# LitLeo/3m-asr-inference

Hardware: AMD Instinct MI355X
Metric: encoder frames/sec, 18Lx32e Conformer-MoE, 206-frame utterance (higher is better)
Workload: dtype f32; 1 GPU; 18-layer 32-expert fp32 (v_mfma_f32_16x16x4_f32), batch=1x206 frames per GPU, all experts local (BASELINE.json configs[1]); layers=18, experts=32, frames=206, batch_per_gpu=1, parallelism=replicas x1, streams_per_gpu=4, hip_graph=True, kernels_per_forward=263, fold_pos_proj=True, routing=balanced, route_mode=staged, packed_rows=False, fork_embed=auto

## Files before the change

### 3m-asr-inference_amd/csrc/gemm.hip

```cpp
#include "common.h"
#include "gemm_epilogue.h"
#include "kernels.h"

#ifdef M3_GEMM_DIAG
#define M3_GDIAG(...) __VA_ARGS__
#else
#define M3_GDIAG(...)
#endif

namespace m3 {

M3_GDIAG(__device__ unsigned long long g_gemm_dbg[2048 * 8];)

enum { LN_NONE = GEMM_LN_NONE, LN_EPI = GEMM_LN_EPI, LN_PRO = GEMM_LN_PRO };

template <int MT, bool GLU, int NW, bool CONV, int LN, int NBUF, bool ACCI = false, bool WF = false>
__device__ __forceinline__ void gemm_f32_body(const GemmParams& p, const int bid) {
  static_assert(!WF || (!CONV && !ACCI), "fragment-ordered W: plain A only");
  constexpr int NT = GLU ? 2 : 1;
  constexpr int G = gemm_group_steps(MT, NT, NW);
  constexpr int I0 = ACCI ? G / 2 : 0;
  static_assert(!ACCI || (MT == 1 && !GLU && !CONV && NBUF == 1 && G % 2 == 0), "acc_init: the one-group 16-row concat form only");
  constexpr int RW = (16 * MT) / NW;
  static_assert(RW >= 1, "more waves than rows");
  __shared__ float red[NW][MT * NT][256];
  __shared__ float stats[16 * MT][2];
  __shared__ float rsum[LN == LN_EPI ? NW : 1][16 * MT][2];
  __shared__ __attribute__((aligned(16))) float ln_g[LN == LN_PRO ? 1024 : 4], ln_b[LN == LN_PRO ? 1024 : 4];

  M3_GDIAG(unsigned long long dg[8]; dg[0] = __builtin_amdgcn_s_memtime();)
  asm volatile("" ::"s"(p.A), "s"(p.lda), "s"(p.W), "s"(p.bias), "s"(p.Y), "s"(p.ldy), "s"(p.M), "s"(p.N), "s"(p.K), "s"(p.mode),
               "s"(p.n_tiles), "s"(p.m_tiles), "s"(p.xcd_swizzle), "s"(p.m_dev), "s"(p.resid), "s"(p.ldr), "s"(p.act), "s"(p.alpha),
               "s"(p.mask_in), "s"(p.mask_out), "s"(p.row_len), "s"(p.rows_per_batch), "s"(p.sig_col0));
  if (ACCI) asm volatile("" ::"s"(p.acc_init));
  if (LN == LN_EPI) asm volatile("" ::"s"(p.ln_wsum), "s"(p.ln_wbeta), "s"(p.ln_eps));
  if (LN == LN_PRO) asm volatile("" ::"s"(p.ln_gamma), "s"(p.ln_beta), "s"(p.ln_eps), "s"(p.ln_out), "s"(p.ld_ln_out), "s"(p.ln_on_a2));
  if (!CONV) asm volatile("" ::"s"(p.A2), "s"(p.lda2), "s"(p.K1));
  if (CONV) asm volatile("" ::"s"(p.conv_T1), "s"(p.conv_F1), "s"(p.conv_T2), "s"(p.conv_F2), "s"(p.conv_C));
  const int lane = threadIdx.x & 63, wave = threadIdx.x >> 6;
  const int col = lane & 15, kq = lane >> 4;
  const int Nout = GLU ? (p.N >> 1) : p.N;

  int n_tile, m_tile;
  {
    const int id = bid;
    if (p.xcd_swizzle) {
      const int j = id >> 3;
      m_tile = j % p.m_tiles;
      n_tile = (j / p.m_tiles) * 8 + (id & 7);
    } else {
      n_tile = id % p.n_tiles;
      m_tile = id / p.n_tiles;
    }
  }
  const int n0 = n_tile * 16;
  const int m0 = m_tile * (16 * MT);
  if (p.m_dev != nullptr && m0 > *p.m_dev) return;
  const int ln_k0 = p.ln_on_a2 ? p.K1 : 0;
  const int Kl = p.K - ln_k0;

  const float* arow[MT];
  const float* arow2[MT];
#pragma unroll
  for (int mt = 0; mt < MT; ++mt) {
    const int m = min(m0 + 16 * mt + col, p.M - 1);
    arow2[mt] = nullptr;
    if (CONV) {
      const int f2 = m % p.conv_F2;
      const int t2 = (m / p.conv_F2) % p.conv_T2;
      const int b = m / (p.conv_F2 * p.conv_T2);
      arow[mt] = p.A + ((size_t)(b * p.conv_T1 + 2 * t2) * p.conv_F1 + 2 * f2) * p.conv_C + 4 * kq;
    } else {
      arow[mt] = p.A + (size_t)m * p.lda + 4 * kq;
      if (p.mode == GEMM_A_CONCAT2) arow2[mt] = p.A2 + (size_t)m * p.lda2 + 4 * kq;
    }
  }
  const float* wrow[NT];
#pragma unroll
  for (int t = 0; t < NT; ++t)
    wrow[t] = WF ? p.W + (size_t)(n_tile + t * (Nout >> 4)) * ((size_t)p.K << 4) + 4 * lane
                 : p.W + (size_t)min(n0 + t * Nout + col, p.N - 1) * p.K + 4 * kq;

  f32x4 acc[MT][NT];
#pragma unroll
  for (int mt = 0; mt < MT; ++mt)
#pragma unroll
    for (int t = 0; t < NT; ++t) acc[mt][t] = f32x4{0.f, 0.f, 0.f, 0.f};
  constexpr bool DUAL = MT * NT <= 2;
  f32x4 acc2[MT][NT];
#pragma unroll
  for (int mt = 0; mt < MT; ++mt)
#pragma unroll
    for (int t = 0; t < NT; ++t) acc2[mt][t] = f32x4{0.f, 0.f, 0.f, 0.f};
  float s1[MT], s2[MT];
#pragma unroll
  for (int mt = 0; mt < MT; ++mt) s1[mt] = s2[mt] = 0.f;

  const int nsteps = p.K >> 4;
  auto a_offset = [&](int k) -> int {
    if (CONV) {
      const int seg = k / p.conv_C, c = k - seg * p.conv_C;
      const int kh = seg / 3, kw = seg - kh * 3;
      return (kh * p.conv_F1 + kw) * p.conv_C + c;
    }
    return k;
  };

  f32x4 wbuf[NBUF][G][NT], abuf[NBUF][G][MT];
  auto load_group = [&](int g, int buf) {
#pragma unroll
    for (int i = I0; i < G; ++i) {
      const int s = min(wave + NW * (G * g + i), nsteps - 1);
      const int k = s << 4;
#pragma unroll
      for (int t = 0; t < NT; ++t) wbuf[buf][i][t] = ldg4_w(wrow[t] + (WF ? (s << 8) : k));
      const bool second = ACCI || (!CONV && p.mode == GEMM_A_CONCAT2 && k >= p.K1);
      const int off = second ? (k - p.K1) : a_offset(k);
#pragma unroll
      for (int mt = 0; mt < MT; ++mt) abuf[buf][i][mt] = ldg4((second ? arow2[mt] : arow[mt]) + off);
    }
  };

  const int ngroups = (nsteps + NW * G - 1) / (NW * G);
  M3_GDIAG(dg[1] = __builtin_amdgcn_s_memtime();)
  f32x4 ln_v[16];
  auto load_stat_rows = [&](int c) {
    const int l16 = lane & 15;
    const int rloc = wave * RW + 4 * c + (lane >> 4);
    const int m = min(m0 + min(rloc, 16 * MT - 1), p.M - 1);
    const float* row = (p.ln_on_a2 ? p.A2 : p.A) + (size_t)m * (p.ln_on_a2 ? p.lda2 : p.lda);
#pragma unroll
    for (int j = 0; j < 8; ++j) ln_v[j] = ldg4(row + min(4 * (l16 + 16 * j), Kl - 4));
    if (Kl > 512) {
#pragma unroll
      for (int j = 8; j < 16; ++j) ln_v[j] = ldg4(row + min(4 * (l16 + 16 * j), Kl - 4));
    } else {
#pragma unroll
      for (int j = 8; j < 16; ++j) ln_v[j] = f32x4{0.f, 0.f, 0.f, 0.f};
    }
  };
  if (LN == LN_PRO && ACCI) load_stat_rows(0);
  load_group(0, 0);
  if (ACCI) {
    const float* pre = p.acc_init + ((size_t)((m_tile * p.n_tiles + n_tile) * NW + wave) * 2) * 256 + 4 * lane;
    acc[0][0] = ldg4(pre);
    acc2[0][0] = ldg4(pre + 256);
  }
  M3_GDIAG(dg[2] = __builtin_amdgcn_s_memtime();)
  const int ep_mt = wave;
  const bool is_ep = wave < MT;
  const int ep_n = n0 + col;
  float bias0 = 0.f, bias1 = 0.f, wsum0 = 0.f, wsum1 = 0.f, wbeta0 = 0.f, wbeta1 = 0.f, res[4] = {0.f, 0.f, 0.f, 0.f};
  if (is_ep && ep_n < Nout) {
    if (p.bias) {
      bias0 = p.bias[ep_n];
      if (GLU) bias1 = p.bias[ep_n + Nout];
    }
    if (LN == LN_EPI) {
      wsum0 = p.ln_wsum[ep_n];
      if (GLU) wsum1 = p.ln_wsum[ep_n + Nout];
      if (p.mask_in) {
        wbeta0 = p.ln_wbeta[ep_n];
        if (GLU) wbeta1 = p.ln_wbeta[ep_n + Nout];
      }
    }
    if (p.resid) {
#pragma unroll
      for (int r = 0; r < 4; ++r) {
        const int m = min(m0 + 16 * ep_mt + 4 * kq + r, p.M - 1);
        res[r] = p.resid[(size_t)m * p.ldr + ep_n];
      }
    }
  }
  bool pad4[4] = {false, false, false, false};
  if (is_ep && (p.mask_in || p.mask_out)) {
#pragma unroll
    for (int r = 0; r < 4; ++r) {
      const int m = min(m0 + 16 * ep_mt + 4 * kq + r, p.M - 1);
      pad4[r] = gemm_row_padded(p, m);
    }
  }


  float a_mean[MT], a_rstd[MT];
  float* ln_out_row[MT];
#pragma unroll
  for (int mt = 0; mt < MT; ++mt) {
    a_mean[mt] = 0.f;
    a_rstd[mt] = 1.f;
    ln_out_row[mt] = nullptr;
  }
  if (LN == LN_PRO) {
    for (int k = threadIdx.x * 4; k < Kl; k += 256 * NW) {
      *reinterpret_cast<f32x4*>(&ln_g[k]) = ldg4(p.ln_gamma + k);
      *reinterpret_cast<f32x4*>(&ln_b[k]) = ldg4(p.ln_beta + k);
    }
    const int q = lane >> 4, l16 = lane & 15;
    const int nj = (Kl + 63) >> 6;
    for (int c = 0; c < (RW + 3) / 4; ++c) {
      const int rloc = wave * RW + 4 * c + q;
      const bool row_on = (4 * c + q) < RW;
      f32x4 v[16];
      if (!(ACCI && c == 0)) load_stat_rows(c);
#pragma unroll
      for (int j = 0; j < 16; ++j) {
        const int k = 4 * (l16 + 16 * j);
        const f32x4 t = ln_v[j];
        const bool in = j < nj && k < Kl;
        v[j] = f32x4{in ? t[0] : 0.f, in ? t[1] : 0.f, in ? t[2] : 0.f, in ? t[3] : 0.f};
      }
      float sum = 0.f;
#pragma unroll
      for (int j = 0; j < 16; ++j) sum += (v[j][0] + v[j][1]) + (v[j][2] + v[j][3]);
      const float mean = group16_sum(sum) / (float)Kl;
      float sq = 0.f;
#pragma unroll
      for (int j = 0; j < 16; ++j) {
        const int k = 4 * (l16 + 16 * j);
        const float on = (j < nj && k < Kl) ? 1.f : 0.f;
#pragma unroll
        for (int e = 0; e < 4; ++e) {
          const float d = (v[j][e] - mean) * on;
          sq += d * d;
        }
      }
      const float var = group16_sum(sq) / (float)Kl;
      if (row_on && l16 == 0) {
        stats[rloc][0] = mean;
        stats[rloc][1] = rsqrtf(var + p.ln_eps);
      }
    }
    __syncthreads();
#pragma unroll
    for (int mt = 0; mt < MT; ++mt) {
      a_mean[mt] = stats[16 * mt + col][0];
      a_rstd[mt] = stats[16 * mt + col][1];
      const int m = m0 + 16 * mt + col;
      if (p.ln_out != nullptr && n_tile == 0 && m < p.M) ln_out_row[mt] = p.ln_out + (size_t)m * p.ld_ln_out + 4 * kq;
    }
  }

  auto compute_group = [&](int g, int buf) {
#pragma unroll
    for (int i = I0; i < G; ++i) {
      const int s = wave + NW * (G * g + i);
      if (s < nsteps) {
        const int k = s << 4;
        const bool in_ln = k >= ln_k0;
        f32x4 g4, b4;
        if (LN == LN_PRO && in_ln) {
          g4 = *reinterpret_cast<const f32x4*>(&ln_g[(k - ln_k0) + 4 * kq]);
          b4 = *reinterpret_cast<const f32x4*>(&ln_b[(k - ln_k0) + 4 * kq]);
        }
#pragma unroll
        for (int mt = 0; mt < MT; ++mt) {
          f32x4 a = abuf[buf][i][mt];
          if (LN == LN_PRO && in_ln) {
#pragma unroll
            for (int j = 0; j < 4; ++j) a[j] = (a[j] - a_mean[mt]) * a_rstd[mt] * g4[j] + b4[j];
            if (ln_out_row[mt] != nullptr) stg4(ln_out_row[mt] + (k - ln_k0), a);
          }
          if (LN == LN_EPI && in_ln) {
            s1[mt] += (a[0] + a[1]) + (a[2] + a[3]);
            s2[mt] += (a[0] * a[0] + a[1] * a[1]) + (a[2] * a[2] + a[3] * a[3]);
          }
#pragma unroll
          for (int t = 0; t < NT; ++t) {
            if (DUAL) {
#pragma unroll
              for (int j = 0; j < 4; j += 2) {
                acc[mt][t] = mfma16(a[j], wbuf[buf][i][t][j], acc[mt][t]);
                acc2[mt][t] = mfma16(a[j + 1], wbuf[buf][i][t][j + 1], acc2[mt][t]);
              }
            } else {
#pragma unroll
              for (int j = 0; j < 4; ++j) acc[mt][t] = mfma16(a[j], wbuf[buf][i][t][j], acc[mt][t]);
            }
          }
        }
      }
    }
  };

  M3_GDIAG(asm volatile("s_waitcnt vmcnt(0)" ::: "memory"); dg[3] = __builtin_amdgcn_s_memtime();)
  if (NBUF == 1) {
    compute_group(0, 0);
  } else {
    for (int g = 0; g < ngroups; g += 2) {
      if (g + 1 < ngroups) load_group(g + 1, NBUF - 1);
      compute_group(g, 0);
      if (g + 1 < ngroups) {
        if (g + 2 < ngroups) load_group(g + 2, 0);
        compute_group(g + 1, NBUF - 1);
      }
    }
  }

  if (DUAL) {
#pragma unroll
    for (int mt = 0; mt < MT; ++mt)
#pragma unroll
      for (int t = 0; t < NT; ++t) acc[mt][t] += acc2[mt][t];
  }
  M3_GDIAG(asm volatile("s_nop 15\n\ts_nop 15" ::: "memory"); dg[4] = __builtin_amdgcn_s_memtime();)
#pragma unroll
  for (int mt = 0; mt < MT; ++mt)
#pragma unroll
    for (int t = 0; t < NT; ++t)
#pragma unroll
      for (int r = 0; r < 4; ++r) red[wave][mt * NT + t][r * 64 + lane] = acc[mt][t][r];
  if (LN == LN_EPI) {
#pragma unroll
    for (int mt = 0; mt < MT; ++mt) {
      float a1 = s1[mt], a2 = s2[mt];
      a1 += __shfl_xor(a1, 16, 64);
      a2 += __shfl_xor(a2, 16, 64);
      a1 += __shfl_xor(a1, 32, 64);
      a2 += __shfl_xor(a2, 32, 64);
      if (kq == 0) {
        rsum[wave][16 * mt + col][0] = a1;
        rsum[wave][16 * mt + col][1] = a2;
      }
    }
  }
  __syncthreads();
  M3_GDIAG(dg[5] = __builtin_amdgcn_s_memtime();)

  if (is_ep) {
    const int mt = ep_mt;
    f32x4 v[NT];
#pragma unroll
    for (int t = 0; t < NT; ++t)
#pragma unroll
      for (int r = 0; r < 4; ++r) {
        float sum = 0.f;
#pragma unroll
        for (int w = 0; w < NW; w += 4)
          sum += (red[w][mt * NT + t][r * 64 + lane] + red[w + 1][mt * NT + t][r * 64 + lane]) +
                 (red[w + 2][mt * NT + t][r * 64 + lane] + red[w + 3][mt * NT + t][r * 64 + lane]);
        v[t][r] = sum;
      }
    if (ep_n < Nout) {
#pragma unroll
      for (int r = 0; r < 4; ++r) {
        const int row = 16 * mt + 4 * kq + r;
        const int m = m0 + row;
        if (m >= p.M) continue;
        float y0 = v[0][r], y1 = v[NT - 1][r];
        const bool pad = pad4[r];
        if (LN != LN_EPI && p.mask_in && pad) y0 = y1 = 0.f;
        float mean = 0.f, rstd = 1.f;
        if (LN == LN_EPI) {
          float t1 = 0.f, t2 = 0.f;
#pragma unroll
          for (int w = 0; w < NW; ++w) {
            t1 += rsum[w][row][0];
            t2 += rsum[w][row][1];
          }
          ln_mean_rstd(t1, t2, Kl, p.ln_eps, mean, rstd);
        }
        float y = gemm_epilogue<GLU, LN == LN_EPI>(y0, y1, bias0, bias1, wsum0, wsum1, wbeta0, wbeta1, mean, rstd, pad, res[r], p);
        if (!GLU && p.sig_col0 >= 0 && n0 >= p.sig_col0) y = sigmoidf(y);
        p.Y[(size_t)m * p.ldy + ep_n] = y;
      }
    }
  }
  M3_GDIAG(dg[6] = __builtin_amdgcn_s_memtime();
           asm volatile("s_waitcnt vmcnt(0)" ::: "memory");
           dg[7] = __builtin_amdgcn_s_memtime();
           if (lane == 0 && wave == 0 && bid < 2048) {
             unsigned long long* o = g_gemm_dbg + (size_t)bid * 8;
             for (int i = 0; i < 8; ++i) o[i] = dg[i];
             const unsigned hw = __builtin_amdgcn_s_getreg((31 << 11) | 4), xcc = __builtin_amdgcn_s_getreg((31 << 11) | 20);
             o[7] = (dg[7] & 0xffffffffffull) | ((unsigned long long)(hw & 0xffff) << 40) | ((unsigned long long)(xcc & 0xf) << 56);
           })
}

template <int MT, bool GLU, int NW, bool CONV, int LN, int NBUF, bool ACCI = false, bool WF = false>
__global__ __launch_bounds__(64 * NW) void gemm_f32_kernel(const GemmParams p) {
  gemm_f32_body<MT, GLU, NW, CONV, LN, NBUF, ACCI, WF>(p, (int)blockIdx.x);
}

struct RouterPrefixArgs {
  const float* A; int lda; int M, N, K;
  int n_tiles, m_tiles, xcd_swizzle;
  const int32_t* m_dev;
  float* prefix; long layer_floats; int layer0;
  const float* w[kRouterPrefixMaxLayers];
};
template <int NW>
__global__ __launch_bounds__(64 * NW) void router_embed_prefix_kernel(const RouterPrefixArgs a) {
  constexpr int H = gemm_group_steps(1, 1, NW) / 2;
  asm volatile("" ::"s"(a.A), "s"(a.lda), "s"(a.M), "s"(a.N), "s"(a.K), "s"(a.n_tiles), "s"(a.m_tiles), "s"(a.xcd_swizzle), "s"(a.m_dev),
               "s"(a.prefix), "s"(a.layer_floats), "s"(a.layer0));
  const int lane = threadIdx.x & 63, wave = threadIdx.x >> 6;
  const int col = lane & 15, kq = lane >> 4;
  const int layer = a.layer0 + (int)blockIdx.y;
  int n_tile, m_tile;
  {
    const int id = (int)blockIdx.x;
    if (a.xcd_swizzle) {
      const int j = id >> 3;
      m_tile = j % a.m_tiles;
      n_tile = (j / a.m_tiles) * 8 + (id & 7);
    } else {
      n_tile = id % a.n_tiles;
      m_tile = id / a.n_tiles;
    }
  }
  const int n0 = n_tile * 16, m0 = m_tile * 16;
  if (a.m_dev != nullptr && m0 > *a.m_dev) return;
  const float* arow = a.A + (size_t)min(m0 + col, a.M - 1) * a.lda + 4 * kq;
  const float* wrow = a.w[layer] + (size_t)min(n0 + col, a.N - 1) * a.K + 4 * kq;
  f32x4 wb[H], ab[H];
#pragma unroll
  for (int i = 0; i < H; ++i) {
    const int k = (wave + NW * i) << 4;
    wb[i] = ldg4_w(wrow + k);
    ab[i] = ldg4(arow + k);
  }
  f32x4 acc = f32x4{0.f, 0.f, 0.f, 0.f}, acc2 = f32x4{0.f, 0.f, 0.f, 0.f};
#pragma unroll
  for (int i = 0; i < H; ++i)
#pragma unroll
    for (int j = 0; j < 4; j += 2) {
      acc = mfma16(ab[i][j], wb[i][j], acc);
      acc2 = mfma16(ab[i][j + 1], wb[i][j + 1], acc2);
    }
  float* o = a.prefix + (size_t)layer * a.layer_floats + ((size_t)((m_tile * a.n_tiles + n_tile) * NW + wave) * 2) * 256 + 4 * lane;
  stg4(o, acc);
  stg4(o + 256, acc2);
}

size_t router_prefix_floats(const GemmPlan& plan) { return (size_t)plan.m_tiles * plan.n_tiles * plan.nw * 2 * 256; }

int launch_router_embed_prefix(const GemmPlan& plan, const GemmParams& p, const float* const* w, int layer0, int n_layers, float* prefix,
                               hipStream_t stream) {
  M3_REQUIRE(plan.launches == 1 && plan.kernel == GemmKernel::SkinnyF32 && p.acc_init != nullptr && (plan.nw == 4 || plan.nw == 8),
             "router prefix: the consumer's plan does not take an accumulator prefix");
  M3_REQUIRE(layer0 >= 0 && n_layers > 0 && layer0 + n_layers <= kRouterPrefixMaxLayers && prefix != nullptr, "router prefix: bad layer range");
  RouterPrefixArgs a;
  a.A = p.A; a.lda = p.lda; a.M = p.M; a.N = p.N; a.K = p.K;
  a.n_tiles = plan.n_tiles; a.m_tiles = plan.m_tiles; a.xcd_swizzle = plan.xcd_swizzle;
  a.m_dev = p.m_dev; a.prefix = prefix; a.layer_floats = (long)router_prefix_floats(plan); a.layer0 = layer0;
  for (int l = 0; l < kRouterPrefixMaxLayers; ++l) a.w[l] = (l >= layer0 && l < layer0 + n_layers) ? w[l] : nullptr;
  const dim3 grid(plan.n_tiles * plan.m_tiles, n_layers);
  if (plan.nw == 8) hipLaunchKernelGGL((router_embed_prefix_kernel<8>), grid, dim3(512), 0, stream, a);
  else hipLaunchKernelGGL((router_embed_prefix_kernel<4>), grid, dim3(256), 0, stream, a);
  M3_LAUNCH_CHECK();
  return 0;
}
template <int MT, bool GLU, int NW, int LN, bool WF = false>
__global__ __launch_bounds__(64 * NW) void gemm_f32_dual_kernel(const GemmParams p0, const GemmParams p1, const int n0) {
  if ((int)blockIdx.x < n0) {
    if ((int)blockIdx.x < p0.n_tiles * p0.m_tiles) gemm_f32_body<MT, GLU, NW, false, LN, 1, false, WF>(p0, (int)blockIdx.x);
  } else {
    gemm_f32_body<MT, GLU, NW, false, LN, 1, false, WF>(p1, (int)blockIdx.x - n0);
  }
}

int launch_gemm_f32_dual(const GemmLaunch& a, const GemmLaunch& b, hipStream_t stream) {
  M3_REQUIRE(gemm_dual_fusable(a, b), "gemm dual: the two problems do not share an instantiation");
  GemmParams q[2] = {a.p, b.p};
  const GemmPlan& pa = a.plan;
  const GemmPlan* const plans[2] = {&a.plan, &b.plan};
  for (int i = 0; i < 2; ++i) {
    q[i].n_tiles = plans[i]->n_tiles; q[i].m_tiles = plans[i]->m_tiles; q[i].xcd_swizzle = plans[i]->xcd_swizzle;
  }
  const int n0 = (int)align_up((size_t)q[0].n_tiles * q[0].m_tiles, 8);
  dim3 grid(n0 + q[1].n_tiles * q[1].m_tiles);
#define M3_DUAL(GLU_, NW_, LN_)                                                                                             \
  do {                                                                                                                      \
    if (q[0].w_frag) hipLaunchKernelGGL((gemm_f32_dual_kernel<1, GLU_, NW_, LN_, true>), grid, dim3(64 * NW_), 0, stream, q[0], q[1], n0); \
    else hipLaunchKernelGGL((gemm_f32_dual_kernel<1, GLU_, NW_, LN_>), grid, dim3(64 * NW_), 0, stream, q[0], q[1], n0);    \
  } while (0)
  if (pa.glu) {
    if (pa.nw == 8) { if (pa.ln == LN_EPI) M3_DUAL(true, 8, LN_EPI); else M3_DUAL(true, 8, LN_NONE); }
    else { if (pa.ln == LN_EPI) M3_DUAL(true, 4, LN_EPI); else M3_DUAL(true, 4, LN_NONE); }
  } else {
    if (pa.nw == 8) { if (pa.ln == LN_EPI) M3_DUAL(false, 8, LN_EPI); else M3_DUAL(false, 8, LN_NONE); }
    else { if (pa.ln == LN_EPI) M3_DUAL(false, 4, LN_EPI); else M3_DUAL(false, 4, LN_NONE); }
  }
#undef M3_DUAL
  M3_LAUNCH_CHECK();
  return 0;
}

int launch_gemm_f32_skinny(const GemmPlan& plan, const GemmParams& pin, hipStream_t stream) {
  GemmParams p = pin;
  p.n_tiles = plan.n_tiles; p.m_tiles = plan.m_tiles; p.xcd_swizzle = plan.xcd_swizzle;
  dim3 grid(p.n_tiles * p.m_tiles);
  const int mt = plan.mt, nw = plan.nw, ln = plan.ln;
  if (p.acc_init != nullptr) {
    if (nw == 8) hipLaunchKernelGGL((gemm_f32_kernel<1, false, 8, false, LN_PRO, 1, true>), grid, dim3(512), 0, stream, p);
    else hipLaunchKernelGGL((gemm_f32_kernel<1, false, 4, false, LN_PRO, 1, true>), grid, dim3(256), 0, stream, p);
    M3_LAUNCH_CHECK();
    return 0;
  }

#define M3_GEMM_LAUNCH(MT_, GLU_, NW_, CONV_, LN_)                                                              \
  do {                                                                                                          \
    constexpr bool kWf = !(CONV_);         \
    if (p.w_frag && plan.nbuf == 1)                                                                              \
      hipLaunchKernelGGL((gemm_f32_kernel<MT_, GLU_, NW_, CONV_, LN_, 1, false, kWf>), grid, dim3(64 * NW_), 0, stream, p); \
    else if (p.w_frag)                                                                                           \
      hipLaunchKernelGGL((gemm_f32_kernel<MT_, GLU_, NW_, CONV_, LN_, 2, false, kWf>), grid, dim3(64 * NW_), 0, stream, p); \
    else if (plan.nbuf == 1)                                                                                    \
      hipLaunchKernelGGL((gemm_f32_kernel<MT_, GLU_, NW_, CONV_, LN_, 1>), grid, dim3(64 * NW_), 0, stream, p); \
    else                                                                                                        \
      hipLaunchKernelGGL((gemm_f32_kernel<MT_, GLU_, NW_, CONV_, LN_, 2>), grid, dim3(64 * NW_), 0, stream, p); \
  } while (0)
#define M3_GEMM_MT(GLU_, NW_, CONV_, LN_)                                                              \
  do {                                                                                                 \
    if (mt == 1) M3_GEMM_LAUNCH(1, GLU_, NW_, CONV_, LN_);                                             \
    else if (mt == 2) M3_GEMM_LAUNCH(2, GLU_, NW_, CONV_, LN_);                                        \
    else M3_GEMM_LAUNCH(4, GLU_, NW_, CONV_, LN_);                                                     \
  } while (0)
#define M3_GEMM_LN(GLU_, NW_)                                                                          \
  do {                                                                                                 \
    if (ln == LN_EPI) M3_GEMM_MT(GLU_, NW_, false, LN_EPI);                                            \
    else if (ln == LN_PRO) M3_GEMM_MT(GLU_, NW_, false, LN_PRO);                                       \
    else M3_GEMM_MT(GLU_, NW_, false, LN_NONE);                                                        \
  } while (0)
  if (plan.conv) {
    if (nw == 16) M3_GEMM_MT(false, 16, true, LN_NONE); else if (nw == 8) M3_GEMM_MT(false, 8, true, LN_NONE);
    else M3_GEMM_MT(false, 4, true, LN_NONE);
  } else if (nw == 16) {
    M3_GEMM_MT(false, 16, false, LN_NONE);
  } else if (plan.glu) {
    if (nw == 8) M3_GEMM_LN(true, 8); else M3_GEMM_LN(true, 4);
  } else {
    if (nw == 8) M3_GEMM_LN(false, 8); else M3_GEMM_LN(false, 4);
  }
#undef M3_GEMM_LN
#undef M3_GEMM_MT
#undef M3_GEMM_LAUNCH
  M3_LAUNCH_CHECK();
  return 0;
}

}

#ifdef M3_GEMM_DIAG
extern "C" int m3_debug_gemm_read(void* dst, size_t bytes) {
  return (int)hipMemcpyFromSymbol(dst, HIP_SYMBOL(m3::g_gemm_dbg), bytes < sizeof(m3::g_gemm_dbg) ? bytes : sizeof(m3::g_gemm_dbg));
}
#endif
```

### 3m-asr-inference_amd/csrc/gemm_epilogue.h

```cpp
#pragma once
#include "common.h"
#include "kernels.h"

namespace m3 {

__device__ __forceinline__ bool gemm_row_padded(const GemmParams& p, int m) {
  return (m % p.rows_per_batch) >= p.row_len[m / p.rows_per_batch];
}

__device__ __forceinline__ void ln_mean_rstd(float sum, float sumsq, int K, float eps, float& mean, float& rstd) {
  mean = sum / (float)K;
  const float var = fmaxf(sumsq / (float)K - mean * mean, 0.f);
  rstd = rsqrtf(var + eps);
}

template <int W>
__device__ __forceinline__ float lanes_sum(float v) {
  static_assert(W == 8 || W == 16 || W == 32, "8, 16 or 32 lanes");
  v += dpp_mov<0xB1>(v);
  v += dpp_mov<0x4E>(v);
  v += dpp_mov<0x141>(v);
  if (W >= 16) v += dpp_mov<0x140>(v);
  if (W == 32) v += __shfl_xor(v, 16, 64);
  return v;
}

template <bool GLU, bool LN>
__device__ __forceinline__ float gemm_epilogue(float y0, float y1, float bias0, float bias1, float wsum0, float wsum1, float wbeta0,
                                               float wbeta1, float mean, float rstd, bool pad, float res, const GemmParams& p) {
  if (LN) {
    if (p.mask_in && pad) {
      y0 = -wbeta0;
      y1 = -wbeta1;
    } else {
      y0 = rstd * (y0 - mean * wsum0);
      y1 = rstd * (y1 - mean * wsum1);
    }
  }
  float y = y0 + bias0;
  if (GLU) y = y * sigmoidf(y1 + bias1);
  if (p.act == ACT_RELU) y = fmaxf(y, 0.f);
  if (p.act == ACT_SILU) y = silu(y);
  if (p.mask_out && pad) y = 0.f;
  y *= p.alpha;
  if (p.resid) y += res;
  return y;
}

}
```

### 3m-asr-inference_amd/csrc/kernels.h

```cpp
#pragma once
#include <hip/hip_runtime.h>
#include <stdint.h>

#include "../../include/m3asr.h"

namespace m3 {

enum { ACT_NONE = 0, ACT_RELU = 1, ACT_SILU = 2, ACT_GLU = 3 };
enum { GEMM_A_PLAIN = 0, GEMM_A_CONCAT2 = 1, GEMM_A_CONV3X3S2 = 2 };

struct GemmParams {
  const float* A = nullptr; int lda = 0;
  const float* A2 = nullptr; int lda2 = 0; int K1 = 0;
  const float* W = nullptr;
  int w_bf16 = 0;
  const float* bias = nullptr;
  float* Y = nullptr; int ldy = 0;
  int M = 0, N = 0, K = 0;
  int mode = GEMM_A_PLAIN;
  const float* ln_gamma = nullptr; const float* ln_beta = nullptr; float ln_eps = 0.f;
  const float* ln_wsum = nullptr; const float* ln_wbeta = nullptr;
  int ln_on_a2 = 0;
  float* ln_out = nullptr; int ld_ln_out = 0;
  const int32_t* row_len = nullptr; int rows_per_batch = 0;
  int mask_in = 0, mask_out = 0;
  int conv_T1 = 0, conv_F1 = 0, conv_T2 = 0, conv_F2 = 0, conv_C = 0;
  int act = ACT_NONE;
  float alpha = 1.f;
  const float* resid = nullptr; int ldr = 0;
  const int32_t* grp_acc = nullptr; int grp_E = 0; const int32_t* grp_pos = nullptr; int w_sliced = 0;
  const float* w_scale = nullptr;
  int a_bf16 = 0, y_bf16 = 0; void* Yb = nullptr; int ldyb = 0;
  float* Yb_stats = nullptr; const float* ln_stats = nullptr; int ln_stat_parts = 0;
  const int32_t* m_dev = nullptr;
  const int32_t* y_rows = nullptr;
  const int32_t* conv_len = nullptr;
  int sig_col0 = -1;
  const float* acc_init = nullptr;
  int w_frag = 0;
  int n_tiles = 0, m_tiles = 0, xcd_swizzle = 0;
};
enum { GEMM_LN_NONE = 0, GEMM_LN_EPI = 1, GEMM_LN_PRO = 2 };
enum class GemmKernel { SkinnyF32, SkinnyBf16, TiledF32, TiledBf16, DmaBf16, SplitKF32 };
struct GemmPlan {
  GemmKernel kernel;
  const char* label;
  int launches;
  bool glu, conv; int ln;
  int mt, nw, nbuf;
  bool dual_ok;
  int bm, bn, bk;
  int stages;
  int m_tiles, n_tiles, xcd_swizzle;
  int splits; size_t ws_bytes;
  char reason[192];
};
GemmPlan plan_gemm(const GemmParams& p, size_t workspace_bytes_available);
struct GemmLaunch { GemmParams p; GemmPlan plan; float* ws = nullptr; };
GemmLaunch gemm_launch(const GemmParams& p, float* ws, size_t ws_bytes);
int launch_gemm(const GemmLaunch& g, hipStream_t stream);
bool gemm_dual_fusable(const GemmLaunch& a, const GemmLaunch& b);
int launch_gemm_f32_dual(const GemmLaunch& a, const GemmLaunch& b, hipStream_t stream);
constexpr int kRouterPrefixMaxLayers = 64;
size_t router_prefix_floats(const GemmPlan& plan);
int launch_router_embed_prefix(const GemmPlan& plan, const GemmParams& p, const float* const* w, int layer0, int n_layers, float* prefix,
                               hipStream_t stream);
constexpr int gemm_group_steps(int MT, int NT, int NW) {
  if (NW == 16) return MT == 1 ? (NT == 1 ? 4 : 2) : (MT == 2 ? 2 : 1);
  if (NW == 8) return MT == 1 ? 8 : (MT == 2 ? (NT == 1 ? 6 : 4) : (NT == 1 ? 3 : 2));
  return MT == 1 ? 8 : (MT == 2 ? 6 : 4);
}
constexpr int gemm16_group_steps(int MT, int NW) { return NW == 16 ? 2 : (MT == 4 ? 2 : 4); }
int launch_gemm_f32_skinny(const GemmPlan& plan, const GemmParams& p, hipStream_t stream);
int launch_gemm_bf16w_skinny(const GemmPlan& plan, const GemmParams& p, hipStream_t stream);
int launch_gemm_f32_tiled(const GemmPlan& plan, const GemmParams& p, hipStream_t stream);
int launch_gemm_bf16w_tiled(const GemmPlan& plan, const GemmParams& p, hipStream_t stream);
int launch_gemm_bf16_dma(const GemmPlan& plan, const GemmParams& p, hipStream_t stream);
int launch_gemm_f32_splitk(const GemmPlan& plan, const GemmParams& p, float* ws, hipStream_t stream);
bool gemm_splitk_dual_fusable(const GemmLaunch& a, const GemmLaunch& b);
int launch_gemm_f32_splitk_dual(const GemmLaunch& a, const GemmLaunch& b, hipStream_t stream, int which = 3);
int init_gemm_f32_splitk_kernels();
int init_gemm_bf16_tiled_kernels();
int init_gemm_f32_tiled_kernels();
int init_gemm_bf16_dma_kernels();
constexpr int kXbStatParts = 4;
int launch_row_stats_bf16(const void* xb, int rows, int D, float* stats, hipStream_t stream);

int launch_moe_index(const int32_t* gate_idx, int S, int E, int32_t* mapping, int32_t* acc_hist,
                     int32_t* pos, hipStream_t stream);
int launch_moe_gate_index(const float* logits, int width, const int32_t* row_len, int rows_per_batch, int S,
                          int32_t* gate_idx, float* gate_value, int32_t* mapping, int32_t* acc_hist, int32_t* pos,
                          hipStream_t stream);
int launch_moe_route(const float* x, int ldx, int D, const float* wx, const float* wsum, const float* bias,
                     const float* eall, int ld_e, float ln_eps, const int32_t* row_len, int rows_per_batch, int S, int E,
                     int32_t* gate_idx, float* gate_value, int32_t* mapping, int32_t* acc_hist, int32_t* pos,
                     hipStream_t stream);
bool moe_router_supports(int De, int D, int N);
bool moe_router_fuses_top1(int N);
int init_moe_router_kernels();
int launch_moe_router(const float* emb, int lde, int De, const float* x, int ldx, int D, const float* W, const float* bias,
                      const float* gamma, const float* beta, float eps, float* xn, int ldxn, float* Y, int ldy, int M, int N,
                      const int32_t* m_dev, hipStream_t stream, int32_t* gate_idx = nullptr, float* gate_val = nullptr,
                      const int32_t* row_len = nullptr, int rows_per_batch = 0, void* xq = nullptr, float* xq_scale = nullptr);
int launch_local_scatter(const void* x, const int32_t* mapping, int S, int row_bytes, void* out, hipStream_t stream);
int launch_local_gather(const void* buf, const int32_t* mapping, int S, int row_bytes, void* out, hipStream_t stream);

int launch_ep_send_map(const int32_t* gate_idx, const int32_t* mapping, const int32_t* acc_hist, int S, int world, int e_loc,
                       int capacity, int32_t* map_send, void* wire, int row_bytes, hipStream_t stream, int32_t* overflow = nullptr);
int launch_ep_send_rows(const int32_t* gate_idx, const int32_t* mapping, const int32_t* acc_hist, int S, int world, int e_loc,
                        int capacity, int32_t* map_send, const void* x, void* wire, int row_bytes, hipStream_t stream, int32_t* overflow = nullptr);
int launch_ep_recv_gate(const void* wire, int world, int e_loc, int capacity, int row_bytes, int32_t* gate_recv,
                        hipStream_t stream);

#ifndef M3_EXPERT_SLICE
#define M3_EXPERT_SLICE 64
#endif
constexpr int kExpertSliceW16 = 64;
constexpr int kExpertSlice = M3_EXPERT_SLICE;
size_t expert_ffn_slab_bytes(int S, int D, int F);
enum class ExpertWeights { F32, BF16, FP8, FP8A8, MXFP4 };
enum class ExpertKernel { SlabF32, TiledF32, SlabBf16, TiledBf16, G256Bf16, SlabW8, TiledW8, FusedFp8, SlabW4, TiledW4 };
struct ExpertFfnPlan {
  ExpertWeights weights; ExpertKernel kernel;
  const char* label;
  int launches, slices;
  int fsplit;
  size_t h_off, rows_off, xb_off;
  float* rows(float* slab) const { return (float*)((char*)slab + rows_off); }
};
enum { EXPERT_NORM_IN_KERNEL = 1,
       EXPERT_SCATTER_ROWS = 2 };
ExpertFfnPlan plan_expert_ffn(ExpertWeights w, int S, int E, int D, int F, unsigned flags = 0);
enum { EXPERT_W_REF = 0, EXPERT_W2_SLICED = 1, EXPERT_W_FRAG = 2 };
struct ExpertFfnArgs { const float* x; int ldx; const int32_t *pos, *acc_hist; const void *w1, *w2; const float *s1, *s2, *b1, *b2;
                       int w2_sliced; float h_scale; float* slab; const float *ln_gamma, *ln_beta; float ln_eps;
                       const void* xq; const float* xq_scale; int32_t* fs_dev; float* y_scatter; };
int launch_expert_ffn(const ExpertFfnPlan& plan, int S, int E, int D, int F, const ExpertFfnArgs& a, hipStream_t stream);
int init_expert_ffn_kernels();
int launch_expert_ffn_f32_slab(const float* x, int ldx, const int32_t* pos, const int32_t* acc_hist, int S, int E,
                               int D, int F, const float* w1, const float* b1, const float* w2, int w2_sliced, float* slab,
                               const float* ln_gamma, const float* ln_beta, float ln_eps, hipStream_t stream);
int init_expert_ffn_f32_tiled_kernels();
int launch_expert_tiled_f32(const float* x, int ldx, const int32_t* pos, const int32_t* acc_hist, int S, int E,
                            int D, int F, const float* w1, const float* b1, const float* w2, int w2_sliced,
                            float* hbuf, float* ybuf, hipStream_t stream);
int init_expert_ffn_bf16_kernels();
int launch_expert_ffn_bf16w_slab(const float* x, int ldx, const int32_t* pos, const int32_t* acc_hist, int S, int E,
                                 int D, int F, const void* w1, const float* b1, const void* w2, int w2_sliced, float* slab,
                                 hipStream_t stream);
int init_expert_ffn_w8_kernels();
int launch_expert_ffn_w8_slab(const float* x, int ldx, const int32_t* pos, const int32_t* acc_hist, int S, int E, int D, int F,
                              const void* w1, const float* s1, const float* b1, const void* w2, const float* s2, int w2_sliced,
                              float* slab, hipStream_t stream);
int init_expert_ffn_w4_kernels();
int launch_expert_ffn_w4_slab(const float* x, int ldx, const int32_t* pos, const int32_t* acc_hist, int S, int E, int D, int F,
                              const void* w1, const void* s1, const float* b1, const void* w2, const void* s2, int w2_sliced,
                              float* slab, hipStream_t stream);
constexpr int kExpertFusedFp8MaxSplit = 4;
int expert_ffn_fused_fp8_fsplit(int S, int E, int D, int F);
int init_expert_ffn_fused_fp8_kernels();
int launch_expert_ffn_fused_fp8(const float* x, int ldx, const int32_t* pos, const int32_t* acc_hist, int S, int E, int D, int F,
                                const void* w1, const float* s1, const float* b1, const void* w2, const float* s2, int w2_sliced,
                                float h_scale, int fsplit, float* ybuf, hipStream_t stream, const void* xq = nullptr,
                                const float* xq_scale = nullptr, int32_t* fs_dev = nullptr);
int launch_quantize_rows_e4m3(const float* x, int ldx, int S, int D, void* xq, float* scale, hipStream_t stream);
int launch_expert_tiled_w16(int w_fp8, const float* x, int ldx, const int32_t* pos, const int32_t* acc_hist, int S, int E,
                            int D, int F, const void* w1, const float* s1, const float* b1, const void* w2, const float* s2,
                            int w2_sliced, void* hbuf, float* ybuf, hipStream_t stream, const float* b2 = nullptr,
                            float* y_scatter = nullptr);
bool expert_ffn_f32_self_routing(int S, int E);
int launch_expert_route_ffn_f32(const float* x, int ldx, const float* logits, const int32_t* row_len, int rows_per_batch, int S, int E,
                                int D, int F, const float* w1, const float* b1, const float* w2, int w2_sliced, const float* b2,
                                float* slab, int32_t* gate_idx, float* gate_value, int32_t* mapping, int32_t* acc_hist, int32_t* pos,
                                hipStream_t stream, const float* ln_gamma = nullptr, const float* ln_beta = nullptr, float ln_eps = 0.f);
bool expert_gemm_g256_takes(int S, int E, int D, int F);
int init_expert_gemm_g256_kernels();
int launch_rows_to_bf16(const float* x, int ldx, int S, int D, void* xb, hipStream_t stream);
int launch_expert_ffn_bf16_g256(const void* xb, int ldxb, const int32_t* pos, const int32_t* acc_hist, int S, int E, int D, int F,
                                const void* w1, const float* b1, const void* w2, int w2_sliced, void* hbuf, float* ybuf,
                                hipStream_t stream);
int launch_moe_combine(const float* slab, int n_slices, const int32_t* mapping, const int32_t* gate_idx,
                       const float* gate_value, const float* b2, const float* resid, float alpha,
                       const float* ln_gamma, const float* ln_beta, float ln_eps, float* out, int S, int D,
                       hipStream_t stream, void* out_bf16 = nullptr, float* out_stats = nullptr,
                       const int32_t* n_slices_dev = nullptr);

int launch_layernorm(const float* x, const float* gamma, const float* beta, float eps, float* y, int rows, int D,
                     hipStream_t stream, void* y_bf16 = nullptr, float* y_stats = nullptr, const float* gamma2 = nullptr,
                     const float* beta2 = nullptr, float eps2 = 0.f, float* y2 = nullptr);
int launch_softmax_top1(const float* logits, int ld, const int32_t* row_len, int rows_per_batch, int S, int E,
                        int32_t* idx, float* value, hipStream_t stream);
int launch_att_masked_softmax(const float* scores, const int32_t* len, int B, int H, int T1, int T2, float scale,
                              float* out, hipStream_t stream);
int launch_masked_fill(const float* x, const int32_t* len, int B, int C, int T, float fill, float* y,
                       hipStream_t stream);
int launch_glu(const float* x, int outer, int C, int inner, float* y, hipStream_t stream);
int launch_scale(const float* x, float scale, float* y, size_t n, hipStream_t stream);
int launch_mask_conv2d_sample(const int32_t* len_in, int B, int left_padding, int stride, int32_t* len_out,
                              hipStream_t stream);
int launch_subsample_lens(const int32_t* len_in, int B, int32_t* len_out, hipStream_t stream);
int launch_add(const float* a, const float* b, float* y, size_t n, hipStream_t stream);
int launch_binary_bcast(const float* a, const float* b, float* y, const int64_t* shape, const int64_t* sa,
                        const int64_t* sb, int nd, int op, hipStream_t stream);
int launch_unary(const float* x, float* y, size_t n, int act, hipStream_t stream);
int launch_permute(const float* x, float* y, const int64_t* out_shape, const int64_t* in_strides, int nd,
                   hipStream_t stream);
int launch_concat_last(const float* a, int da, const float* b, int db, float* y, size_t rows, hipStream_t stream);
int launch_softmax_lastdim(const float* x, float* y, size_t rows, int n, hipStream_t stream);
int launch_bmm(const float* a, const float* b, float* c, int batch, int M, int N, int K, int64_t sa, int64_t sb,
               int trans_b, hipStream_t stream);

struct AttArgs {
  const void* qkv = nullptr; int ldq = 0; const float* pmat = nullptr; int ldp = 0; const float *pos_u = nullptr, *pos_v = nullptr;
  const int32_t* row_len = nullptr; int B = 0, T = 0, H = 0, dk = 0; float scale = 1.f; void* out = nullptr; int ldo = 0, out_bf16 = 0;
  const int32_t* row0 = nullptr; int chunk = 0, left_chunks = 0;
  int rows_bf16 = 0;
  int streaming = 0; float* hist = nullptr; int cap = 0; const int32_t* step = nullptr;
  int slot_max_chunks = -1;
};
int launch_relpos_attention(const AttArgs& a, hipStream_t stream);
bool relpos_attention_dual_fusable(const AttArgs& a, const AttArgs& b);
int launch_relpos_attention_dual(const AttArgs& a, const AttArgs& b, hipStream_t stream);
bool relpos_attention_bf16_supports(int T, int dk);
int init_relpos_attention_bf16_kernels();

int launch_pad2d(const float* x, size_t outer, int H, int W, int pre_h, int post_h, int pre_w, int post_w, float* y, hipStream_t stream);
int launch_advance_counter(int32_t* counter, int by, hipStream_t stream);
int launch_fill_rows(const float* row, int D, float* out, size_t rows, hipStream_t stream);
int launch_advance_slots(int32_t* pos, int32_t* status, int32_t* frames, const int32_t* chunk_len, int B, int C, int max_chunks,
                         hipStream_t stream);
constexpr int kMaxStreamBlocks = 64;
struct SlotResetArgs {
  int32_t *pos = nullptr, *status = nullptr, *frames = nullptr;
  const int32_t* slots = nullptr; int n = 0;
  int B = 0, K = 0, D = 0, n_blocks = 0;
  float* conv[kMaxStreamBlocks];
  const float* fill[kMaxStreamBlocks];
};
int launch_reset_slots(const SlotResetArgs& a, hipStream_t stream);
int launch_slot_positions(const int32_t* status, const int32_t* frames, int B, int32_t* out, hipStream_t stream);
struct DwArgs {
  const float *z = nullptr, *w_kc = nullptr, *bias = nullptr, *gamma = nullptr, *beta = nullptr; float eps = 1e-5f;
  int B = 0, T = 0, D = 0, K = 0; float* out = nullptr; int out_bf16 = 0;
  const int32_t *pad_of = nullptr, *row0 = nullptr, *row_len = nullptr;
  const float* causal_left_fill = nullptr;
  int glu_ldz = 0;
  int glu_sig = 0;
  int streaming = 0; float* cache_pair = nullptr; const int32_t *step = nullptr, *chunk_len = nullptr;
  int slot_max_chunks = -1;
};
int launch_dwconv_ln_silu(const DwArgs& a, hipStream_t stream);
bool dwconv_glu_in_supports(int D, int K, bool causal_or_stream, int out_bf16, int ldz);
bool dwconv_dual_fusable(const DwArgs& a, const DwArgs& b);
int launch_dwconv_ln_silu_dual(const DwArgs& a, const DwArgs& b, hipStream_t stream);
int launch_pack_plan(int32_t* len, int B, int T, int32_t* row0, int32_t* pad_of, hipStream_t stream,
                     const int32_t* feat_len = nullptr);
int launch_unpack_rows(const float* in, const int32_t* row0, int B, int T, int n, float* out, hipStream_t stream);
struct Conv1Args {
  const float *feat = nullptr, *w9c = nullptr, *bias = nullptr, *cmvn_mean = nullptr, *cmvn_istd = nullptr;
  int B = 0, T = 0, idim = 0, C = 0; float* out = nullptr; int relu = 1, out_bf16 = 0;
  const int32_t* feat_len = nullptr; int32_t* lens_out = nullptr;
  int in_ch = 1;
};
int launch_conv1_relu(const Conv1Args& a, hipStream_t stream);
bool conv1_dual_fusable(const Conv1Args& a, const Conv1Args& b);
int launch_conv1_relu_dual(const Conv1Args& a, const Conv1Args& b, hipStream_t stream);
int launch_cmvn(const float* x, const int32_t* len, const float* mean, const float* istd, int B, int T, int D,
                float* y, hipStream_t stream);
int launch_log_softmax_bias(const float* x, const float* bias, float* y, size_t rows, int n, hipStream_t stream);
int launch_ctc_greedy(const float* logits, const int32_t* len, int B, int T, int V, int blank, int32_t* frame_ids,
                      int32_t* tokens, int32_t* n_tokens, hipStream_t stream);
int launch_ctc_topk(const float* logits, size_t rows, int V, int k, float* top_logp, int32_t* top_idx, hipStream_t stream);
int ctc_prefix_beam_search_host(const float* top_logp, const int32_t* top_idx, int T, int k, int beam, int blank,
                                int32_t* hyp_tokens, int32_t* hyp_len, float* hyp_score, int32_t* n_hyps);
int launch_ctc_argmax(const float* logits, size_t rows, int V, int32_t* ids, hipStream_t stream);
size_t ctc_beam_state_size(const m3_ctc_beam_desc* d);
int launch_ctc_beam_reset(const m3_ctc_beam_desc* d, void* state, size_t bytes, hipStream_t stream,
                          const int32_t* slots = nullptr, int n = 0);
int launch_ctc_beam_advance(const m3_ctc_beam_desc* d, void* state, size_t bytes, const float* top_logp, const int32_t* top_idx,
                            int T_chunk, const int32_t* n_frames, hipStream_t stream);
int launch_ctc_beam_nbest(const m3_ctc_beam_desc* d, const void* state, size_t bytes, int32_t* hyp_tokens, int32_t* hyp_len,
                          float* hyp_score, int32_t* n_hyps, hipStream_t stream);
size_t ctc_align_workspace_size(const m3_ctc_align_desc* d);
int launch_ctc_align_emit(const m3_ctc_align_desc* d, const float* logits, int ldl, const int32_t* row0, const int32_t* n_frames,
                          const int32_t* tokens, const int32_t* tok0, float* emit, hipStream_t stream);
int launch_ctc_align_path(const m3_ctc_align_desc* d, const float* emit, const int32_t* n_frames, const int32_t* tokens,
                          const int32_t* tok0, void* workspace, size_t ws_bytes, float* score, int32_t* status, int32_t* state,
                          int32_t* tok_start, int32_t* tok_end, int32_t* tok_peak, float* tok_logp, hipStream_t stream);
constexpr int32_t kCtxMagic = 0x5843334d;
constexpr int kCtxMaxGraphs = 1024, kCtxMaxStates = 65536;
constexpr size_t kCtxMaxBytes = (size_t)64 << 20;
enum { CTX_MAGIC = 0, CTX_G = 1, CTX_V = 2, CTX_WORDS = 3, CTX_HDR_WORDS = 4 };
enum { CTXG_STATES = 0, CTXG_A = 1, CTXG_CLS = 2, CTXG_NEXT = 3, CTXG_DELTA = 4, CTXG_POT = 5, CTXG_WORDS = 8 };
struct CtxGraph {
  const int32_t* cls;
  const int32_t* next;
  const float* delta;
  const float* pot;
  int n_states, A, V;
};
__host__ __device__ inline bool ctx_graph_view(const int32_t* image, long long words, int g, CtxGraph* out) {
  if (image == nullptr || words < CTX_HDR_WORDS || image[CTX_MAGIC] != kCtxMagic) return false;
  const long long G = image[CTX_G], V = image[CTX_V];
  if (G < 0 || G > kCtxMaxGraphs || V < 1 || CTX_HDR_WORDS + G * CTXG_WORDS > words || g < 0 || g >= G) return false;
  const int32_t* h = image + CTX_HDR_WORDS + (long long)g * CTXG_WORDS;
  const long long ns = h[CTXG_STATES], A = h[CTXG_A], first = CTX_HDR_WORDS + G * CTXG_WORDS;
  if (ns < 1 || ns > kCtxMaxStates || A < 1 || A > V + 1 || A > kCtxMaxStates) return false;
  const long long off[4] = {h[CTXG_CLS], h[CTXG_NEXT], h[CTXG_DELTA], h[CTXG_POT]};
  const long long len[4] = {V, ns * A, ns * A, ns};
  for (int i = 0; i < 4; ++i)
    if (off[i] < first || off[i] > words || len[i] > words - off[i]) return false;
  out->cls = image + off[0];
  out->next = image + off[1];
  out->delta = (const float*)(image + off[2]);
  out->pot = (const float*)(image + off[3]);
  out->n_states = (int)ns;
  out->A = (int)A;
  out->V = (int)V;
  return true;
}
int ctc_context_validate(const void* image, size_t bytes, int V);
int ctc_prefix_beam_search_ctx_host(const float* top_logp, const int32_t* top_idx, int T, int k, int beam, int blank,
                                    const void* image, size_t image_bytes, int graph, int32_t* hyp_tokens, int32_t* hyp_len,
                                    float* hyp_score, float* hyp_bonus, int32_t* hyp_state, int32_t* n_hyps);
size_t ctc_beam_ctx_state_size(const m3_ctc_beam_desc* d);
int launch_ctc_beam_ctx_reset(const m3_ctc_beam_desc* d, void* state, size_t bytes, hipStream_t stream,
                              const int32_t* slots = nullptr, int n = 0);
int launch_ctc_beam_ctx_advance(const m3_ctc_beam_desc* d, void* state, size_t bytes, const void* image, size_t image_bytes,
                                const int32_t* graph_of, const float* top_logp, const int32_t* top_idx, int T_chunk,
                                const int32_t* n_frames, hipStream_t stream);
int launch_ctc_beam_ctx_nbest(const m3_ctc_beam_desc* d, const void* state, size_t bytes, const void* image, size_t image_bytes,
                              const int32_t* graph_of, int32_t* hyp_tokens, int32_t* hyp_len, float* hyp_score,
                              float* hyp_bonus, int32_t* n_hyps, hipStream_t stream);
constexpr int32_t kLmMagic = 0x4d4c334d;
constexpr int32_t kLmVersion = 1;
constexpr int kLmMaxOrder = 8, kLmMaxStates = 1 << 26;
constexpr size_t kLmMaxBytes = (size_t)1 << 30;
enum { LM_MAGIC = 0, LM_VERSION = 1, LM_V = 2, LM_ORDER = 3, LM_STATES = 4, LM_ARCS = 5, LM_START = 6, LM_UNK = 7, LM_TABLES = 8,
       LM_WORDS = 17, LM_HDR_WORDS = 20 };
enum { LMT_UNI_LOGP = 0, LMT_UNI_NEXT, LMT_ARC_BEGIN, LMT_ARC_TOK, LMT_ARC_NEXT, LMT_ARC_LOGP, LMT_BO_STATE, LMT_BO_WEIGHT,
       LMT_FINAL, LMT_COUNT };
struct LmView {
  const float* uni_logp;
// ... 200 lines not shown
```

Before: 170,700 frames/s.

## Trim skinny GEMM scalar/VGPR pressure: magic division, spread epilogue, occupancy bounds

Replaces the integer div/mod in tile decoding and padding-row checks with host-precomputed multiply-shift reciprocals. It packs the scalar-pinning asm operands into 64-bit pairs and adds a one-run flag so the row_len lookup skips the division. For single-M-tile kernels the epilogue is spread across four waves, each handling one row, instead of one wave handling four. It also adds a min-waves launch bound for specific configurations. The goal is fewer SALU/VALU cycles and registers per block so occupancy rises, at the risk of register spilling under the tighter launch bounds.

```diff
diff --git a/3m-asr-inference_amd/csrc/gemm.hip b/3m-asr-inference_amd/csrc/gemm.hip
--- a/3m-asr-inference_amd/csrc/gemm.hip
+++ b/3m-asr-inference_amd/csrc/gemm.hip
@@ -29,14 +29,21 @@
   __shared__ __attribute__((aligned(16))) float ln_g[LN == LN_PRO ? 1024 : 4], ln_b[LN == LN_PRO ? 1024 : 4];
 
   M3_GDIAG(unsigned long long dg[8]; dg[0] = __builtin_amdgcn_s_memtime();)
-  asm volatile("" ::"s"(p.A), "s"(p.lda), "s"(p.W), "s"(p.bias), "s"(p.Y), "s"(p.ldy), "s"(p.M), "s"(p.N), "s"(p.K), "s"(p.mode),
-               "s"(p.n_tiles), "s"(p.m_tiles), "s"(p.xcd_swizzle), "s"(p.m_dev), "s"(p.resid), "s"(p.ldr), "s"(p.act), "s"(p.alpha),
-               "s"(p.mask_in), "s"(p.mask_out), "s"(p.row_len), "s"(p.rows_per_batch), "s"(p.sig_col0));
-  if (ACCI) asm volatile("" ::"s"(p.acc_init));
-  if (LN == LN_EPI) asm volatile("" ::"s"(p.ln_wsum), "s"(p.ln_wbeta), "s"(p.ln_eps));
-  if (LN == LN_PRO) asm volatile("" ::"s"(p.ln_gamma), "s"(p.ln_beta), "s"(p.ln_eps), "s"(p.ln_out), "s"(p.ld_ln_out), "s"(p.ln_on_a2));
-  if (!CONV) asm volatile("" ::"s"(p.A2), "s"(p.lda2), "s"(p.K1));
-  if (CONV) asm volatile("" ::"s"(p.conv_T1), "s"(p.conv_F1), "s"(p.conv_T2), "s"(p.conv_F2), "s"(p.conv_C));
+  {
+    auto pk = [](int lo, int hi) { return (unsigned long long)(unsigned)lo | ((unsigned long long)(unsigned)hi << 32); };
+    constexpr bool EPI = LN == LN_EPI, PRO = LN == LN_PRO;
+    asm volatile("" ::"s"(p.A), "s"(p.W), "s"(p.bias), "s"(p.Y), "s"(p.m_dev), "s"(p.resid), "s"(p.row_len),
+                 "s"(pk(p.lda, p.ldy)), "s"(pk(p.M, p.N)), "s"(pk(p.K, p.mode)), "s"(pk(p.n_tiles, p.m_tiles)),
+                 "s"(pk(p.xcd_swizzle, p.ldr)), "s"(pk(p.act, __float_as_int(p.alpha))), "s"(pk(p.mask_in, p.mask_out)),
+                 "s"(pk(p.rows_per_batch, p.sig_col0)), "s"(pk(p.one_run, LN != LN_NONE ? __float_as_int(p.ln_eps) : 0)),
+                 "s"(pk((int)p.div_m_tiles.mul, p.div_m_tiles.shift)), "s"(pk((int)p.div_n_tiles.mul, p.div_n_tiles.shift)),
+                 "s"(pk((int)p.div_rpb.mul, p.div_rpb.shift)),
+                 "s"(ACCI ? p.acc_init : nullptr), "s"(EPI ? p.ln_wsum : PRO ? p.ln_gamma : nullptr),
+                 "s"(EPI ? p.ln_wbeta : PRO ? p.ln_beta : nullptr), "s"(PRO ? p.ln_out : nullptr),
+                 "s"(PRO ? pk(p.ld_ln_out, p.ln_on_a2) : 0ull), "s"(CONV ? nullptr : p.A2),
+                 "s"(CONV ? pk(p.conv_T1, p.conv_F1) : pk(p.lda2, p.K1)), "s"(CONV ? pk(p.conv_T2, p.conv_F2) : 0ull),
+                 "s"(CONV ? p.conv_C : 0));
+  }
   const int lane = threadIdx.x & 63, wave = threadIdx.x >> 6;
   const int col = lane & 15, kq = lane >> 4;
   const int Nout = GLU ? (p.N >> 1) : p.N;
@@ -46,11 +53,12 @@
     const int id = bid;
     if (p.xcd_swizzle) {
       const int j = id >> 3;
-      m_tile = j % p.m_tiles;
-      n_tile = (j / p.m_tiles) * 8 + (id & 7);
+      const int q = gemm_div_by(j, p.div_m_tiles);
+      m_tile = j - q * p.m_tiles;
+      n_tile = q * 8 + (id & 7);
     } else {
-      n_tile = id % p.n_tiles;
-      m_tile = id / p.n_tiles;
+      m_tile = gemm_div_by(id, p.div_n_tiles);
+      n_tile = id - m_tile * p.n_tiles;
     }
   }
   const int n0 = n_tile * 16;
@@ -147,10 +155,16 @@
     acc2[0][0] = ldg4(pre + 256);
   }
   M3_GDIAG(dg[2] = __builtin_amdgcn_s_memtime();)
-  const int ep_mt = wave;
-  const bool is_ep = wave < MT;
+  constexpr bool SPREAD = MT == 1;
+  constexpr int ER = SPREAD ? 1 : 4;
+  static_assert(NW >= 4, "the spread epilogue needs four waves");
+  const int ep_mt = SPREAD ? 0 : wave;
+  const int ep_r0 = SPREAD ? wave : 0;
+  const bool is_ep = SPREAD ? (NW == 4 || wave < 4) : wave < MT;
   const int ep_n = n0 + col;
-  float bias0 = 0.f, bias1 = 0.f, wsum0 = 0.f, wsum1 = 0.f, wbeta0 = 0.f, wbeta1 = 0.f, res[4] = {0.f, 0.f, 0.f, 0.f};
+  float bias0 = 0.f, bias1 = 0.f, wsum0 = 0.f, wsum1 = 0.f, wbeta0 = 0.f, wbeta1 = 0.f, res[ER];
+#pragma unroll
+  for (int r = 0; r < ER; ++r) res[r] = 0.f;
   if (is_ep && ep_n < Nout) {
     if (p.bias) {
       bias0 = p.bias[ep_n];
@@ -166,21 +180,25 @@
     }
     if (p.resid) {
 #pragma unroll
-      for (int r = 0; r < 4; ++r) {
-        const int m = min(m0 + 16 * ep_mt + 4 * kq + r, p.M - 1);
+      for (int r = 0; r < ER; ++r) {
+        const int m = min(m0 + 16 * ep_mt + 4 * kq + ep_r0 + r, p.M - 1);
         res[r] = p.resid[(size_t)m * p.ldr + ep_n];
       }
     }
   }
+  int pad_len = 0;
   bool pad4[4] = {false, false, false, false};
   if (is_ep && (p.mask_in || p.mask_out)) {
-#pragma unroll
-    for (int r = 0; r < 4; ++r) {
-      const int m = min(m0 + 16 * ep_mt + 4 * kq + r, p.M - 1);
-      pad4[r] = gemm_row_padded(p, m);
-    }
-  }
-
+    if (SPREAD) {
+      pad_len = gemm_row_len_request(p, min(m0 + 4 * kq + ep_r0, p.M - 1));
+    } else {
+      int len4[4];
+#pragma unroll
+      for (int r = 0; r < 4; ++r) len4[r] = gemm_row_len_request(p, min(m0 + 16 * ep_mt + 4 * kq + r, p.M - 1));
+#pragma unroll
+      for (int r = 0; r < 4; ++r) pad4[r] = gemm_row_frame(p, min(m0 + 16 * ep_mt + 4 * kq + r, p.M - 1)) >= len4[r];
+    }
+  }
 
   float a_mean[MT], a_rstd[MT];
   float* ln_out_row[MT];
@@ -328,26 +346,27 @@
 
   if (is_ep) {
     const int mt = ep_mt;
-    f32x4 v[NT];
+    float v[NT][ER];
 #pragma unroll
     for (int t = 0; t < NT; ++t)
 #pragma unroll
-      for (int r = 0; r < 4; ++r) {
+      for (int r = 0; r < ER; ++r) {
+        const int e = (ep_r0 + r) * 64 + lane;
         float sum = 0.f;
 #pragma unroll
         for (int w = 0; w < NW; w += 4)
-          sum += (red[w][mt * NT + t][r * 64 + lane] + red[w + 1][mt * NT + t][r * 64 + lane]) +
-                 (red[w + 2][mt * NT + t][r * 64 + lane] + red[w + 3][mt * NT + t][r * 64 + lane]);
+          sum += (red[w][mt * NT + t][e] + red[w + 1][mt * NT + t][e]) + (red[w + 2][mt * NT + t][e] + red[w + 3][mt * NT + t][e]);
         v[t][r] = sum;
       }
     if (ep_n < Nout) {
 #pragma unroll
-      for (int r = 0; r < 4; ++r) {
-        const int row = 16 * mt + 4 * kq + r;
+      for (int r = 0; r < ER; ++r) {
+        const int row = 16 * mt + 4 * kq + ep_r0 + r;
         const int m = m0 + row;
         if (m >= p.M) continue;
         float y0 = v[0][r], y1 = v[NT - 1][r];
-        const bool pad = pad4[r];
+        bool pad = pad4[r];
+        if (SPREAD && (p.mask_in || p.mask_out)) pad = gemm_row_frame(p, m) >= pad_len;
         if (LN != LN_EPI && p.mask_in && pad) y0 = y1 = 0.f;
         float mean = 0.f, rstd = 1.f;
         if (LN == LN_EPI) {
@@ -376,8 +395,12 @@
            })
 }
 
+constexpr int gemm_f32_min_waves(int MT, bool GLU, int NW, bool CONV, int LN, int NBUF, bool WF, bool dual) {
+  return (MT == 1 && !GLU && NW == 8 && LN == LN_NONE && NBUF == 1 && ((dual && WF) || (!dual && CONV))) ? 5 : 1;
+}
+
 template <int MT, bool GLU, int NW, bool CONV, int LN, int NBUF, bool ACCI = false, bool WF = false>
-__global__ __launch_bounds__(64 * NW) void gemm_f32_kernel(const GemmParams p) {
+__global__ __launch_bounds__(64 * NW, gemm_f32_min_waves(MT, GLU, NW, CONV, LN, NBUF, WF, false)) void gemm_f32_kernel(const GemmParams p) {
   gemm_f32_body<MT, GLU, NW, CONV, LN, NBUF, ACCI, WF>(p, (int)blockIdx.x);
 }
 
@@ -451,12 +474,20 @@
   return 0;
 }
 template <int MT, bool GLU, int NW, int LN, bool WF = false>
-__global__ __launch_bounds__(64 * NW) void gemm_f32_dual_kernel(const GemmParams p0, const GemmParams p1, const int n0) {
+__global__ __launch_bounds__(64 * NW, gemm_f32_min_waves(MT, GLU, NW, false, LN, 1, WF, true)) void gemm_f32_dual_kernel(const GemmParams p0, const GemmParams p1, const int n0) {
   if ((int)blockIdx.x < n0) {
     if ((int)blockIdx.x < p0.n_tiles * p0.m_tiles) gemm_f32_body<MT, GLU, NW, false, LN, 1, false, WF>(p0, (int)blockIdx.x);
   } else {
     gemm_f32_body<MT, GLU, NW, false, LN, 1, false, WF>(p1, (int)blockIdx.x - n0);
   }
+}
+
+static void gemm_fill_tiles(GemmParams& p, const GemmPlan& plan) {
+  p.n_tiles = plan.n_tiles; p.m_tiles = plan.m_tiles; p.xcd_swizzle = plan.xcd_swizzle;
+  p.div_m_tiles = gemm_div(plan.m_tiles);
+  p.div_n_tiles = gemm_div(plan.n_tiles);
+  p.div_rpb = gemm_div(p.rows_per_batch > 0 ? p.rows_per_batch : 1);
+  p.one_run = p.rows_per_batch >= p.M ? 1 : 0;
 }
 
 int launch_gemm_f32_dual(const GemmLaunch& a, const GemmLaunch& b, hipStream_t stream) {
@@ -464,9 +495,7 @@
   GemmParams q[2] = {a.p, b.p};
   const GemmPlan& pa = a.plan;
   const GemmPlan* const plans[2] = {&a.plan, &b.plan};
-  for (int i = 0; i < 2; ++i) {
-    q[i].n_tiles = plans[i]->n_tiles; q[i].m_tiles = plans[i]->m_tiles; q[i].xcd_swizzle = plans[i]->xcd_swizzle;
-  }
+  for (int i = 0; i < 2; ++i) gemm_fill_tiles(q[i], *plans[i]);
   const int n0 = (int)align_up((size_t)q[0].n_tiles * q[0].m_tiles, 8);
   dim3 grid(n0 + q[1].n_tiles * q[1].m_tiles);
 #define M3_DUAL(GLU_, NW_, LN_)                                                                                             \
@@ -488,7 +517,7 @@
 
 int launch_gemm_f32_skinny(const GemmPlan& plan, const GemmParams& pin, hipStream_t stream) {
   GemmParams p = pin;
-  p.n_tiles = plan.n_tiles; p.m_tiles = plan.m_tiles; p.xcd_swizzle = plan.xcd_swizzle;
+  gemm_fill_tiles(p, plan);
   dim3 grid(p.n_tiles * p.m_tiles);
   const int mt = plan.mt, nw = plan.nw, ln = plan.ln;
   if (p.acc_init != nullptr) {
diff --git a/3m-asr-inference_amd/csrc/gemm_epilogue.h b/3m-asr-inference_amd/csrc/gemm_epilogue.h
--- a/3m-asr-inference_amd/csrc/gemm_epilogue.h
+++ b/3m-asr-inference_amd/csrc/gemm_epilogue.h
@@ -6,6 +6,15 @@
 
 __device__ __forceinline__ bool gemm_row_padded(const GemmParams& p, int m) {
   return (m % p.rows_per_batch) >= p.row_len[m / p.rows_per_batch];
+}
+
+__device__ __forceinline__ int gemm_div_by(int x, const GemmDiv& d) { return (int)(((unsigned long long)(unsigned)x * d.mul) >> d.shift); }
+
+__device__ __forceinline__ int gemm_row_len_request(const GemmParams& p, int m) {
+  return p.row_len[p.one_run ? 0 : gemm_div_by(m, p.div_rpb)];
+}
+__device__ __forceinline__ int gemm_row_frame(const GemmParams& p, int m) {
+  return p.one_run ? m : m - gemm_div_by(m, p.div_rpb) * p.rows_per_batch;
 }
 
 __device__ __forceinline__ void ln_mean_rstd(float sum, float sumsq, int K, float eps, float& mean, float& rstd) {
diff --git a/3m-asr-inference_amd/csrc/kernels.h b/3m-asr-inference_amd/csrc/kernels.h
--- a/3m-asr-inference_amd/csrc/kernels.h
+++ b/3m-asr-inference_amd/csrc/kernels.h
@@ -8,6 +8,16 @@
 
 enum { ACT_NONE = 0, ACT_RELU = 1, ACT_SILU = 2, ACT_GLU = 3 };
 enum { GEMM_A_PLAIN = 0, GEMM_A_CONCAT2 = 1, GEMM_A_CONV3X3S2 = 2 };
+
+struct GemmDiv { unsigned mul = 0; int shift = 0; };
+inline GemmDiv gemm_div(int d) {
+  int l = 0;
+  while (l < 31 && (1u << l) < (unsigned)d) ++l;
+  GemmDiv r;
+  r.shift = 31 + l;
+  r.mul = (unsigned)(((1ull << r.shift) + (unsigned)d - 1) / (unsigned)d);
+  return r;
+}
 
 struct GemmParams {
   const float* A = nullptr; int lda = 0;
@@ -39,6 +49,8 @@
   const float* acc_init = nullptr;
   int w_frag = 0;
   int n_tiles = 0, m_tiles = 0, xcd_swizzle = 0;
+  int one_run = 0;
+  GemmDiv div_m_tiles, div_n_tiles, div_rpb;
 };
 enum { GEMM_LN_NONE = 0, GEMM_LN_EPI = 1, GEMM_LN_PRO = 2 };
 enum class GemmKernel { SkinnyF32, SkinnyBf16, TiledF32, TiledBf16, DmaBf16, SplitKF32 };
```

Measured after the change: 179,600 frames/s, median of 6. +5.2%, better.
